# lyd405121/ti-raytrace

Measured on AMD Instinct MI355X. Metric: Mrays/s (primary+secondary) at 1024² 100k-tri, 1/2/4/8 GPU + HBM GB/s, higher is better.
Workload: dtype f32

## Files before the change

### ti_raytrace_amd/csrc/tirt_render.hip

```cpp
#include "tirt_trace.h"
#include "tirt_spectral.h"

namespace tirt {

struct ShadeStep {
    bool want_next = false, want_shadow = false, shaded = false;
    v3 next_o = V(0.0f, 0.0f, 0.0f), next_d = next_o, next_thr = next_o, sh_o = next_o, sh_d = next_o, sh_c = next_o;
    float next_pdf = 0.0f, sh_dist = 0.0f; int next_spec = 0, sh_expect = -2;
};
template <unsigned FEAT, bool LIST = false>
TD void shade_path(const SceneView &sc, const TileMap &tm, int P, uint32_t frame_begin, uint32_t seed, int bounce, int last_bounce, int slot,
                   const v3 origin, const v3 direction, const float4 hrec, v3 throughout, v3 &radiance, float brdf_pdf, int perfect_spec, ShadeStep &s)
{
    int f, k; slot_to_frame_pixel(tm, P, slot, f, k);
    const uint32_t pixel = (uint32_t)mapped_pixel<LIST>(tm, k);
    const uint32_t frame = frame_begin + (uint32_t)f;
    const uint32_t dim0 = TM_DIM_BOUNCE0 + TM_DIMS_PER_BOUNCE * (uint32_t)bounce;
    const float t = hrec.x;
    constexpr bool ENV_NEE = (FEAT & SF_ENV_SAMPLE) != 0u;
    constexpr bool ENV_HDR = (FEAT & SF_ENV_HDR) != 0u;
    constexpr bool LIGHT_POW = (FEAT & SF_LIGHT_POWER) != 0u;
    [[maybe_unused]] float p_env = 0.0f;
    if constexpr (ENV_NEE) p_env = sc.light_count == 0 ? 1.0f : env_table(sc).share;
    if (t < INF_VALUE) {
        const int prim_id = __float_as_int(hrec.w);
        int mat_id;
        const HitAttr h = hit_attributes_rec<(FEAT & (SF_TEXTURE | SF_TEXTURE_PARAM)) != 0u>(sc.shade_rec, origin, direction, prim_id, t, hrec.y, hrec.z, mat_id);
        v3 normal = h.nor;
        if constexpr ((FEAT & SF_TEXTURE_PARAM) != 0u) {
            const int nor_id = material_map(sc.material + (size_t)mat_id * MAT_VEC, 9);
            if (nor_id >= 0) normal = tex_normal_rec(sc.tex, sc.shade_rec, nor_id, prim_id, h.tex, normal);
        }
        const v3 fnormal = normal * signf(dot(-direction, h.gnor));
        const float *m = sc.material + (size_t)mat_id * MAT_VEC;
        const v3 mat_color = V(m[2], m[3], m[4]);
        const int mat_type = (int)m[0];
        if (mat_type == MAT_LIGHT) {
            const float fCosTheta = absf(dot(direction, h.gnor));
            if (perfect_spec == 1) {
                radiance = radiance + throughout * mat_color;
            } else {
                const float area = h.area * (float)sc.light_count;
                float light_pdf = (t * t) / (area * fCosTheta);
                if constexpr (LIGHT_POW) light_pdf = (t * t) * (shade_rec_phit(sc.shade_rec, prim_id) / h.area) / fCosTheta;
                if constexpr (ENV_NEE) light_pdf = light_pdf * (1.0f - p_env);
                radiance = radiance + (throughout * power_heuristic(brdf_pdf, light_pdf)) * mat_color;
            }
        } else {
            s.shaded = true;
            v3 reflect_color;
            const int tex_id = (FEAT & SF_TEXTURE) ? material_texture(m) : -1;
            if ((FEAT & SF_TEXTURE) && tex_id >= 0) reflect_color = srgb_to_lrgb(tex_albedo(sc.tex, tex_id, h.tex.x, h.tex.y));
            else reflect_color = V(sc.mat_lrgb[mat_id * 3], sc.mat_lrgb[mat_id * 3 + 1], sc.mat_lrgb[mat_id * 3 + 2]);
            v3 next_dir; float f_or_b = 1.0f, brdf = 1.0f;
            if ((FEAT & SF_GLASS) && mat_type == MAT_GLASS) {
                perfect_spec = 1;
                next_dir = glass_sample(m, direction, normal, tm_rand(seed, pixel, frame, dim0 + TM_SLOT_GLASS), f_or_b);
                brdf = 1.0f; brdf_pdf = 1.0f;
            } else {
                perfect_spec = 0;
                float mp[MAT_VEC];
                const float *md = m;
                if constexpr ((FEAT & SF_TEXTURE_PARAM) != 0u) {
                    for (int w = 0; w < MAT_VEC; w++) mp[w] = m[w];
                    const int metal_id = material_map(m, 8), rough_id = material_map(m, 7);
                    if (metal_id >= 0) mp[5] = tex_metallic(sc.tex, metal_id, h.tex.x, h.tex.y);
                    if (rough_id >= 0) mp[6] = tex_roughness(sc.tex, rough_id, h.tex.x, h.tex.y);
                    md = mp;
                }
                constexpr bool SHARE_SETUP = !(FEAT & SF_GLASS);
                DisneySetup ds;
                if (SHARE_SETUP) ds = disney_setup(md, fnormal, -direction);
                [[maybe_unused]] bool env_taken = false;
                if constexpr (ENV_NEE) {
                    if (tm_rand(seed, pixel, frame, dim0 + TM_SLOT_LIGHT) < p_env) {
                        env_taken = true;
                        const EnvTable et = env_table(sc);
                        const EnvSample es = env_sample(et, sc.env_w, sc.env_h, tm_rand(seed, pixel, frame, dim0 + TM_SLOT_LA), tm_rand(seed, pixel, frame, dim0 + TM_SLOT_LB));
                        const EnvPdf ep = env_pdf(et, sc.env_w, sc.env_h, es.d);
                        const float NdotL = dot(fnormal, es.d);
                        if ((NdotL > 0.0f) & (ep.pdf > 0.0f)) {
                            s.want_shadow = true;
                            float e_pdf;
                            const float e_brdf = SHARE_SETUP ? disney_evaluate_pdf_set(ds, fnormal, -direction, es.d, e_pdf)
                                                             : disney_evaluate_pdf(md, fnormal, -direction, es.d, e_pdf);
                            const float pdf_l = p_env * ep.pdf;
                            v3 c = V(0.0f, 0.0f, 0.0f);
                            int expect = -2;
                            if (e_pdf > 0.0f) {
                                const float w = power_heuristic(pdf_l, e_pdf) / maxf(0.0001f, pdf_l);
                                c = (env_lookup<ENV_HDR>(sc.env, sc.env_w, sc.env_h, ep.tx, ep.ty) * sc.env_power) * w;
                                c = c * throughout;
                                c = c * reflect_color;
                                c = c * e_brdf;
                                c = c * absf(NdotL);
                                const float dr = SHARE_SETUP ? ds.diffuseRatio : 0.5f * (1.0f - md[5]);
                                const float drawn = maxf(0.0f, e_pdf + (dr * (float)(1.0 / 3.1415956)) * (NdotL - 1.0f));
                                c = c * (drawn / e_pdf);
                                expect = -1;
                            }
                            s.sh_o = offset_ray(h.pos, fnormal); s.sh_d = es.d; s.sh_c = c; s.sh_expect = expect; s.sh_dist = ENV_SHADOW_DIST;
                        }
                    }
                }
                if (!env_taken && (!(FEAT & SF_NO_LIGHT) || sc.light_count > 0)) {
                float r_light = tm_rand(seed, pixel, frame, dim0 + TM_SLOT_LIGHT);
                if constexpr (ENV_NEE) r_light = (r_light - p_env) / (1.0f - p_env);
                int lidx = (int)(r_light * (float)sc.light_count);
                if (lidx >= sc.light_count) lidx = sc.light_count - 1;
                [[maybe_unused]] float P_light = 0.0f;
                if constexpr (LIGHT_POW) lidx = light_pick(light_table(sc), sc.light_count, r_light, P_light);
                const float ra = tm_rand(seed, pixel, frame, dim0 + TM_SLOT_LA);
                const float rb = tm_rand(seed, pixel, frame, dim0 + TM_SLOT_LB);
                v3 light_pos, light_normal;
                const LightRec lr = light_sample_rec<LIGHT_POW ? (FEAT & ~(SF_LIGHT_SPOT_LASER | SF_LIGHT_OTHER)) : FEAT>(sc.light_rec, lidx, ra, rb, light_pos, light_normal);
                const float light_choice_pdf = LIGHT_POW ? P_light / lr.area : lr.choice_pdf;
                light_normal = normalized(light_normal);
                v3 light_dir = h.pos - light_pos;
                const float light_dist = norm(light_dir);
                light_dir = light_dir / light_dist;
                const v3 light_emission = lr.emission * light_shape_visible_rec<LIGHT_POW ? (FEAT & ~SF_LIGHT_SPOT_LASER) : FEAT>(lr, light_dir, light_normal, light_dist);
                const float NdotL_surface = dot(fnormal, light_dir);
                const float NdotL_light = dot(light_normal, light_dir);
                if ((NdotL_surface < 0.0f) & (NdotL_light > 0.0f)) {
                    s.want_shadow = true;
                    float e_pdf;
                    const float e_brdf = SHARE_SETUP ? disney_evaluate_pdf_set(ds, fnormal, -direction, -light_dir, e_pdf)
                                                     : disney_evaluate_pdf(md, fnormal, -direction, -light_dir, e_pdf);
                    float light_pdf = light_dist * light_dist * light_choice_pdf / NdotL_light;
                    if constexpr (ENV_NEE) light_pdf = light_pdf * (1.0f - p_env);
                    v3 c = V(0.0f, 0.0f, 0.0f);
                    int expect = -2;
                    if (e_pdf > 0.0f) {
                        const float w = power_heuristic(light_pdf, e_pdf) / maxf(0.0001f, light_pdf);
                        c = light_emission * w;
                        c = c * throughout;
                        c = c * reflect_color;
                        c = c * e_brdf;
                        c = c * absf(NdotL_surface);
                        expect = prim_id;
                    }
                    s.sh_o = light_pos; s.sh_d = light_dir; s.sh_c = c; s.sh_expect = expect; s.sh_dist = light_dist;
                }
                }
                const float r_lobe = tm_rand(seed, pixel, frame, dim0 + TM_SLOT_LOBE), r_1 = tm_rand(seed, pixel, frame, dim0 + TM_SLOT_R1),
                            r_2 = tm_rand(seed, pixel, frame, dim0 + TM_SLOT_R2);
                next_dir = SHARE_SETUP ? disney_sample_set(ds, direction, fnormal, r_lobe, r_1, r_2) : disney_sample(md, direction, fnormal, r_lobe, r_1, r_2);
                f_or_b = 1.0f;
                brdf = SHARE_SETUP ? disney_evaluate_pdf_set(ds, fnormal, -direction, next_dir, brdf_pdf)
                                   : disney_evaluate_pdf(md, fnormal, -direction, next_dir, brdf_pdf);
                brdf *= absf(dot(normal, next_dir));
            }
            const v3 next_origin = offset_ray(h.pos, fnormal * signf(f_or_b));
            if (brdf_pdf > 0.0f) {
                bool alive = true;
                if ((FEAT & SF_GLASS) && f_or_b < 0.0f) {
                    const float extinction = m[6];
                    const float R = tm_exp(-t / extinction);
                    if (tm_rand(seed, pixel, frame, dim0 + TM_SLOT_EXT) >= R) alive = false;
                }
                if (alive) {
                    throughout = throughout * (reflect_color * (brdf / brdf_pdf));
                    s.want_next = !last_bounce;
                    s.next_o = next_origin; s.next_d = next_dir; s.next_thr = throughout;
                    s.next_pdf = brdf_pdf; s.next_spec = perfect_spec;
                }
            }
        }
    } else if ((!(FEAT & SF_ENV) || sc.env_power == 0.0f) && (direction.x - direction.x == 0.0f) && (direction.y - direction.y == 0.0f) &&
               (direction.z - direction.z == 0.0f)) {
        radiance = radiance + throughout * sc.env_power;
    } else if (!(FEAT & SF_ENV)) {
        const float dis = tm_sqrt(direction.x * direction.x + direction.z * direction.z);
        const float big = 3.4028234e38f;
        const bool e_nan = direction.x != direction.x || direction.y != direction.y || direction.z != direction.z ||
                           (absf(direction.x) > big && absf(direction.z) > big) || (absf(direction.y) > big && dis > big);
        const float e1 = e_nan ? tm_nan() : 0.0f;
        radiance = radiance + (V(e1, e1, e1) * throughout) * sc.env_power;
    } else {
        const float dis = tm_sqrt(direction.x * direction.x + direction.z * direction.z);
        const float tx = (tm_atan2(direction.z, direction.x) + PI_SCENE) / PI_SCENE / 2.0f;
        const float ty = tm_atan2(direction.y, dis) / PI_SCENE + 0.5f;
        const v3 e = env_lookup<ENV_HDR>(sc.env, sc.env_w, sc.env_h, tx, ty);
        if constexpr (ENV_NEE) {
            float w = 1.0f;
            if (perfect_spec != 1) w = power_heuristic(brdf_pdf, p_env * env_pdf(env_table(sc), sc.env_w, sc.env_h, direction).pdf);
            radiance = radiance + ((e * throughout) * sc.env_power) * w;
        } else
        radiance = radiance + (e * throughout) * sc.env_power;
    }
}

template <bool LIST>
__global__ void k_generate(PathSoA ps, CameraView cam, TileMap tm, int P, int S, uint32_t frame_begin, uint32_t seed,
                           DevCounters *ctr)
{
    int s = blockIdx.x * blockDim.x + threadIdx.x;
    if (s >= S) return;
    int f, k; slot_to_frame_pixel(tm, P, s, f, k);
    int p = mapped_pixel<LIST>(tm, k);
    int i = p / tm.H, j = p - i * tm.H;
    uint32_t frame = frame_begin + (uint32_t)f;
    float jx = 0.0f, jy = 0.0f;
    if (frame != 0) {
        jx = tm_rand(seed, (uint32_t)p, frame, TM_DIM_JX) - 0.5f;
        jy = tm_rand(seed, (uint32_t)p, frame, TM_DIM_JY) - 0.5f;
    }
    v3 d = camera_ray_direction(cam, i, j, jx, jy);
    __builtin_nontemporal_store(d.x, &ps.dx[s]); __builtin_nontemporal_store(d.y, &ps.dy[s]); __builtin_nontemporal_store(d.z, &ps.dz[s]);
    if (s == 0) atomicAdd(&ctr->paths, (unsigned long long)S);
}

#ifndef SH_BLOCK
#define SH_BLOCK 256
#endif
#ifndef SH_MIN_WAVES
#define SH_MIN_WAVES 5
#endif
#ifndef SH_MIN_WAVES_NARROW
#define SH_MIN_WAVES_NARROW 5
#endif
#ifndef SH_MIN_WAVES_MAPS
#define SH_MIN_WAVES_MAPS 4
#endif
#ifndef SH_MIN_WAVES_ENV
#define SH_MIN_WAVES_ENV 4
#endif
#ifndef SH_MIN_WAVES_POWER
#define SH_MIN_WAVES_POWER 4
#endif
#ifndef SH_MIN_WAVES_HDR
#define SH_MIN_WAVES_HDR 4
#endif
struct ShadeArgs { PathState ps; PathSoA in, out; };
typedef const __attribute__((address_space(4))) ShadeArgs *cold_shade_t;
#define SH_COLD(ca) cold_shade_t ca = (cold_shade_t)__builtin_amdgcn_kernarg_segment_ptr(); asm volatile("" : "+s"(ca))
#define SH_LD(x) __builtin_nontemporal_load(&(x))
#define SH_ST(x, v) __builtin_nontemporal_store((v), &(x))
template <unsigned FEAT, int MIN_WAVES, bool LIST = false>
__global__ __launch_bounds__(SH_BLOCK, MIN_WAVES) void k_shade(ShadeArgs paths_in_kernarg_segment, SceneView sc, TileMap tm, int P,
                                                   uint32_t frame_begin, uint32_t seed, int bounce, int last_bounce,
                                                   const int *count_ptr, int count_fixed, unsigned long long *append_ctr,
                                                   DevCounters *ctr, v3 eye)
{
    __shared__ unsigned s_wcnt[2][SH_BLOCK / 64];
    __shared__ unsigned long long s_base[2];
    const int lane = threadIdx.x & 63, wid = threadIdx.x >> 6;
    const unsigned long long lt_mask = (lane == 0) ? 0ull : (~0ull >> (64 - lane));
    const int count = count_ptr ? *count_ptr : count_fixed;
    const int total = gridDim.x * blockDim.x;
    const int rounds = (count + total - 1) / total;
    unsigned long long n_shaded = 0;
    for (int it = 0; it < rounds; it++) {
        const int q = it * total + blockIdx.x * blockDim.x + threadIdx.x;
        bool live = q < count, want_next = false, want_shadow = false;
        int slot = 0;
        v3 radiance = V(0.0f, 0.0f, 0.0f), next_o = radiance, next_d = radiance, next_thr = radiance;
        v3 sh_o = radiance, sh_d = radiance, sh_c = radiance;
        float next_pdf = 0.0f, sh_dist = 0.0f; int next_spec = 0, sh_expect = -2;
        if (live) {
            const bool first = bounce == 0;
            SH_COLD(ca);
            const int *const c_slot = ca->in.slot; const uint32_t *const c_flags = ca->in.flags; const float4 *const c_hit = ca->ps.hit;
            const float *const c_ox = ca->in.ox, *const c_oy = ca->in.oy, *const c_oz = ca->in.oz, *const c_dx = ca->in.dx, *const c_dy = ca->in.dy, *const c_dz = ca->in.dz;
            const float *const c_tr = ca->in.tr, *const c_tg = ca->in.tg, *const c_tb = ca->in.tb, *const c_rr = ca->in.rr, *const c_rg = ca->in.rg, *const c_rb = ca->in.rb;
            const float *const c_pdf = ca->in.brdf_pdf;
            asm volatile("" :: "s"(c_slot), "s"(c_flags), "s"(c_hit), "s"(c_ox), "s"(c_oy), "s"(c_oz), "s"(c_dx), "s"(c_dy), "s"(c_dz), "s"(c_tr), "s"(c_tg), "s"(c_tb),
                         "s"(c_rr), "s"(c_rg), "s"(c_rb), "s"(c_pdf));
            slot = first ? q : SH_LD(c_slot[q]);
            const v3 origin = first ? eye : V(SH_LD(c_ox[q]), SH_LD(c_oy[q]), SH_LD(c_oz[q]));
            const v3 direction = V(SH_LD(c_dx[q]), SH_LD(c_dy[q]), SH_LD(c_dz[q]));
            typedef float f4nt__ __attribute__((ext_vector_type(4)));
            const f4nt__ hnt__ = __builtin_nontemporal_load((const f4nt__ *)&c_hit[q]);
            const float4 hrec = make_float4(hnt__.x, hnt__.y, hnt__.z, hnt__.w);
            v3 throughout = first ? V(1.0f, 1.0f, 1.0f) : V(SH_LD(c_tr[q]), SH_LD(c_tg[q]), SH_LD(c_tb[q]));
            radiance = first ? V(0.0f, 0.0f, 0.0f) : V(SH_LD(c_rr[q]), SH_LD(c_rg[q]), SH_LD(c_rb[q]));
            float brdf_pdf = first ? 1.0f : SH_LD(c_pdf[q]);
            int perfect_spec = first ? 1 : (int)(SH_LD(c_flags[q]) & 1u);
            ShadeStep ss;
            shade_path<FEAT, LIST>(sc, tm, P, frame_begin, seed, bounce, last_bounce, slot, origin, direction, hrec, throughout, radiance, brdf_pdf, perfect_spec, ss);
            want_next = ss.want_next; want_shadow = ss.want_shadow; if (ss.shaded) n_shaded++;
            next_o = ss.next_o; next_d = ss.next_d; next_thr = ss.next_thr; next_pdf = ss.next_pdf; next_spec = ss.next_spec;
            sh_o = ss.sh_o; sh_d = ss.sh_d; sh_c = ss.sh_c; sh_expect = ss.sh_expect; sh_dist = ss.sh_dist;
        }
        const int par = it & 1;
        const unsigned long long nmask = __ballot(want_next), smask = __ballot(want_shadow);
        if (lane == 0) s_wcnt[par][wid] = (unsigned)__popcll(nmask) | ((unsigned)__popcll(smask) << 16);
        __syncthreads();
        if (threadIdx.x == 0) {
            unsigned tn = 0, tsd = 0;
#pragma unroll
            for (int w = 0; w < SH_BLOCK / 64; w++) { tn += s_wcnt[par][w] & 0xffffu; tsd += s_wcnt[par][w] >> 16; }
            s_base[par] = (tn | tsd) ? atomicAdd(append_ctr, (unsigned long long)tn | ((unsigned long long)tsd << 32)) : 0ull;
        }
        __syncthreads();
        unsigned pn = 0, psd = 0;
#pragma unroll
        for (int w = 0; w < SH_BLOCK / 64; w++) if (w < wid) { pn += s_wcnt[par][w] & 0xffffu; psd += s_wcnt[par][w] >> 16; }
        const unsigned long long bb = s_base[par];
        const int qn = (int)(unsigned)(bb & 0xffffffffull) + (int)pn + __popcll(nmask & lt_mask);
        const int qs = (int)(unsigned)(bb >> 32) + (int)psd + __popcll(smask & lt_mask);
        if (want_next) {
            SH_COLD(ca);
            float *const o_ox = ca->out.ox, *const o_oy = ca->out.oy, *const o_oz = ca->out.oz, *const o_dx = ca->out.dx, *const o_dy = ca->out.dy, *const o_dz = ca->out.dz;
            float *const o_tr = ca->out.tr, *const o_tg = ca->out.tg, *const o_tb = ca->out.tb, *const o_rr = ca->out.rr, *const o_rg = ca->out.rg, *const o_rb = ca->out.rb;
            float *const o_pdf = ca->out.brdf_pdf; uint32_t *const o_flags = ca->out.flags; int *const o_slot = ca->out.slot;
            asm volatile("" :: "s"(o_ox), "s"(o_oy), "s"(o_oz), "s"(o_dx), "s"(o_dy), "s"(o_dz), "s"(o_tr), "s"(o_tg), "s"(o_tb), "s"(o_rr), "s"(o_rg), "s"(o_rb),
                         "s"(o_pdf), "s"(o_flags), "s"(o_slot));
            SH_ST(o_ox[qn], next_o.x); SH_ST(o_oy[qn], next_o.y); SH_ST(o_oz[qn], next_o.z);
            SH_ST(o_dx[qn], next_d.x); SH_ST(o_dy[qn], next_d.y); SH_ST(o_dz[qn], next_d.z);
            SH_ST(o_tr[qn], next_thr.x); SH_ST(o_tg[qn], next_thr.y); SH_ST(o_tb[qn], next_thr.z);
            SH_ST(o_rr[qn], radiance.x); SH_ST(o_rg[qn], radiance.y); SH_ST(o_rb[qn], radiance.z);
            SH_ST(o_pdf[qn], next_pdf); SH_ST(o_flags[qn], (uint32_t)next_spec); SH_ST(o_slot[qn], slot);
        } else if (live) {
            SH_COLD(ca);
            float *const f_r = ca->ps.fr, *const f_g = ca->ps.fg, *const f_b = ca->ps.fb;
            asm volatile("" :: "s"(f_r), "s"(f_g), "s"(f_b));
            SH_ST(f_r[slot], radiance.x); SH_ST(f_g[slot], radiance.y); SH_ST(f_b[slot], radiance.z);
        }
        if (want_shadow) {
            SH_COLD(ca);
            float *const s_ox = ca->ps.sox, *const s_oy = ca->ps.soy, *const s_oz = ca->ps.soz, *const s_dx = ca->ps.sdx, *const s_dy = ca->ps.sdy, *const s_dz = ca->ps.sdz;
            float *const s_cr = ca->ps.scr, *const s_cg = ca->ps.scg, *const s_cb = ca->ps.scb, *const s_dist = ca->ps.sdist;
            int *const s_prim = ca->ps.sprim, *const s_dst = ca->ps.sdst;
            asm volatile("" :: "s"(s_ox), "s"(s_oy), "s"(s_oz), "s"(s_dx), "s"(s_dy), "s"(s_dz), "s"(s_cr), "s"(s_cg), "s"(s_cb), "s"(s_dist), "s"(s_prim), "s"(s_dst));
            SH_ST(s_ox[qs], sh_o.x); SH_ST(s_oy[qs], sh_o.y); SH_ST(s_oz[qs], sh_o.z);
            SH_ST(s_dx[qs], sh_d.x); SH_ST(s_dy[qs], sh_d.y); SH_ST(s_dz[qs], sh_d.z);
            SH_ST(s_cr[qs], sh_c.x); SH_ST(s_cg[qs], sh_c.y); SH_ST(s_cb[qs], sh_c.z);
            SH_ST(s_prim[qs], sh_expect); SH_ST(s_dist[qs], sh_dist);
            SH_ST(s_dst[qs], want_next ? qn : ~slot);
        }
    }
    __shared__ unsigned long long s_shaded;
    if (threadIdx.x == 0) s_shaded = 0ull;
    __syncthreads();
    n_shaded = wave_sum(n_shaded);
    if ((threadIdx.x & 63) == 0 && n_shaded) atomicAdd(&s_shaded, n_shaded);
    __syncthreads();
    if (threadIdx.x == 0 && s_shaded) atomicAdd(&ctr->shaded, s_shaded);
}

template <bool LIST>
__global__ void k_film(PathState ps, TileMap tm, int P, int F, uint32_t frame_begin, float *hdr)
{
    int k = blockIdx.x * blockDim.x + threadIdx.x;
    if (k >= P) return;
    int p = mapped_pixel<LIST>(tm, k);
    float *px = hdr + (size_t)p * 3;
    float r = px[0], g = px[1], b = px[2];
    for (int f = 0; f < F; f++) {
        int s = frame_pixel_to_slot(tm, P, f, k);
        float frame = (float)(int)(frame_begin + (uint32_t)f);
        float coff = 1.0f / (frame + 1.0f);
        r = __builtin_nontemporal_load(&ps.fr[s]) * coff + r * (1.0f - coff);
        g = __builtin_nontemporal_load(&ps.fg[s]) * coff + g * (1.0f - coff);
        b = __builtin_nontemporal_load(&ps.fb[s]) * coff + b * (1.0f - coff);
    }
    px[0] = r; px[1] = g; px[2] = b;
}

template <unsigned FEAT>
__global__ __launch_bounds__(SH_BLOCK, 4) void k_shade_spec(ShadeArgs paths_in_kernarg_segment, SceneView sc, SpecView sp, TileMap tm, int P,
                                                   uint32_t frame_begin, uint32_t seed, int bounce, int last_bounce,
                                                   const int *count_ptr, int count_fixed, unsigned long long *append_ctr,
                                                   DevCounters *ctr, v3 eye)
{
    __shared__ unsigned s_wcnt[2][SH_BLOCK / 64];
    __shared__ unsigned long long s_base[2];
    const int lane = threadIdx.x & 63, wid = threadIdx.x >> 6;
    const unsigned long long lt_mask = (lane == 0) ? 0ull : (~0ull >> (64 - lane));
    const int count = count_ptr ? *count_ptr : count_fixed;
    const int total = gridDim.x * blockDim.x;
    const int rounds = (count + total - 1) / total;
    unsigned long long n_shaded = 0;
    for (int it = 0; it < rounds; it++) {
        const int q = it * total + blockIdx.x * blockDim.x + threadIdx.x;
        bool live = q < count, want_next = false, want_shadow = false;
        int slot = 0;
        f4s radiance = f4_set(0.0f), next_thr = radiance, sh_c = radiance;
        v3 next_o = V(0.0f, 0.0f, 0.0f), next_d = next_o, sh_o = next_o, sh_d = next_o;
        float sh_dist = 0.0f; int sh_expect = -2;
        if (live) {
            const bool first = bounce == 0;
            SH_COLD(ca);
            const int *const c_slot = ca->in.slot; const float4 *const c_hit = ca->ps.hit;
            const float *const c_ox = ca->in.ox, *const c_oy = ca->in.oy, *const c_oz = ca->in.oz, *const c_dx = ca->in.dx, *const c_dy = ca->in.dy, *const c_dz = ca->in.dz;
            const float *const c_tr = ca->in.tr, *const c_tg = ca->in.tg, *const c_tb = ca->in.tb, *const c_rr = ca->in.rr, *const c_rg = ca->in.rg, *const c_rb = ca->in.rb;
            const float *const c_tw = ca->in.brdf_pdf, *const c_rw = (const float *)ca->in.flags;
            asm volatile("" :: "s"(c_slot), "s"(c_hit), "s"(c_ox), "s"(c_oy), "s"(c_oz), "s"(c_dx), "s"(c_dy), "s"(c_dz), "s"(c_tr), "s"(c_tg), "s"(c_tb),
                         "s"(c_rr), "s"(c_rg), "s"(c_rb), "s"(c_tw), "s"(c_rw));
            slot = first ? q : c_slot[q];
            int f, k; slot_to_frame_pixel(tm, P, slot, f, k);
            const uint32_t pixel = (uint32_t)local_to_pixel(tm, k);
            const uint32_t frame = frame_begin + (uint32_t)f;
            const uint32_t dim0 = TM_DIM_BOUNCE0 + TM_DIMS_PER_BOUNCE * (uint32_t)bounce;
            const float Lambda = HERO_LAMBDA_MIN + HERO_LAMBDA_STEP * tm_rand(seed, pixel, frame, TM_DIM_SPEC_LAMBDA);
            const v3 origin = first ? eye : V(c_ox[q], c_oy[q], c_oz[q]);
            const v3 direction = V(c_dx[q], c_dy[q], c_dz[q]);
            typedef float f4nt__ __attribute__((ext_vector_type(4)));
            const f4nt__ hnt__ = __builtin_nontemporal_load((const f4nt__ *)&c_hit[q]);
            const float4 hrec = make_float4(hnt__.x, hnt__.y, hnt__.z, hnt__.w);
            const float t = hrec.x;
            f4s throughout = f4_set(1.0f);
            if (!first) {
                throughout.v[0] = c_tr[q]; throughout.v[1] = c_tg[q]; throughout.v[2] = c_tb[q]; throughout.v[3] = c_tw[q];
                radiance.v[0] = c_rr[q]; radiance.v[1] = c_rg[q]; radiance.v[2] = c_rb[q]; radiance.v[3] = c_rw[q];
            }
            const f4s light_rad = hero_sample(sp.spd[0], Lambda);
            if (t < INF_VALUE) {
                const int prim_id = __float_as_int(hrec.w);
                int mat_id;
                const HitAttr h = hit_attributes_rec(sc.shade_rec, origin, direction, prim_id, t, hrec.y, hrec.z, mat_id);
                const v3 normal = h.nor;
// ... 78 lines not shown
        if (threadIdx.x == 0) {
            unsigned tn = 0, tsd = 0;
#pragma unroll
            for (int w = 0; w < SH_BLOCK / 64; w++) { tn += s_wcnt[par][w] & 0xffffu; tsd += s_wcnt[par][w] >> 16; }
            s_base[par] = (tn | tsd) ? atomicAdd(append_ctr, (unsigned long long)tn | ((unsigned long long)tsd << 32)) : 0ull;
        }
        __syncthreads();
        unsigned pn = 0, psd = 0;
#pragma unroll
        for (int w = 0; w < SH_BLOCK / 64; w++) if (w < wid) { pn += s_wcnt[par][w] & 0xffffu; psd += s_wcnt[par][w] >> 16; }
        const unsigned long long bb = s_base[par];
        const int qn = (int)(unsigned)(bb & 0xffffffffull) + (int)pn + __popcll(nmask & lt_mask);
        const int qs = (int)(unsigned)(bb >> 32) + (int)psd + __popcll(smask & lt_mask);
        if (want_next) {
            SH_COLD(ca);
            float *const o_ox = ca->out.ox, *const o_oy = ca->out.oy, *const o_oz = ca->out.oz, *const o_dx = ca->out.dx, *const o_dy = ca->out.dy, *const o_dz = ca->out.dz;
            float *const o_tr = ca->out.tr, *const o_tg = ca->out.tg, *const o_tb = ca->out.tb, *const o_rr = ca->out.rr, *const o_rg = ca->out.rg, *const o_rb = ca->out.rb;
            float *const o_tw = ca->out.brdf_pdf, *const o_rw = (float *)ca->out.flags; int *const o_slot = ca->out.slot;
            asm volatile("" :: "s"(o_ox), "s"(o_oy), "s"(o_oz), "s"(o_dx), "s"(o_dy), "s"(o_dz), "s"(o_tr), "s"(o_tg), "s"(o_tb), "s"(o_rr), "s"(o_rg), "s"(o_rb),
                         "s"(o_tw), "s"(o_rw), "s"(o_slot));
            o_ox[qn] = next_o.x; o_oy[qn] = next_o.y; o_oz[qn] = next_o.z;
            o_dx[qn] = next_d.x; o_dy[qn] = next_d.y; o_dz[qn] = next_d.z;
            o_tr[qn] = next_thr.v[0]; o_tg[qn] = next_thr.v[1]; o_tb[qn] = next_thr.v[2]; o_tw[qn] = next_thr.v[3];
            o_rr[qn] = radiance.v[0]; o_rg[qn] = radiance.v[1]; o_rb[qn] = radiance.v[2]; o_rw[qn] = radiance.v[3];
            o_slot[qn] = slot;
        } else if (live) {
            SH_COLD(ca);
            float *const f_r = ca->ps.fr, *const f_g = ca->ps.fg, *const f_b = ca->ps.fb, *const f_w = ca->ps.fw;
            asm volatile("" :: "s"(f_r), "s"(f_g), "s"(f_b), "s"(f_w));
            f_r[slot] = radiance.v[0]; f_g[slot] = radiance.v[1]; f_b[slot] = radiance.v[2]; f_w[slot] = radiance.v[3];
        }
        if (want_shadow) {
            SH_COLD(ca);
            float *const s_ox = ca->ps.sox, *const s_oy = ca->ps.soy, *const s_oz = ca->ps.soz, *const s_dx = ca->ps.sdx, *const s_dy = ca->ps.sdy, *const s_dz = ca->ps.sdz;
            float *const s_cr = ca->ps.scr, *const s_cg = ca->ps.scg, *const s_cb = ca->ps.scb, *const s_cw = ca->ps.scw, *const s_dist = ca->ps.sdist;
            int *const s_prim = ca->ps.sprim, *const s_dst = ca->ps.sdst;
            asm volatile("" :: "s"(s_ox), "s"(s_oy), "s"(s_oz), "s"(s_dx), "s"(s_dy), "s"(s_dz), "s"(s_cr), "s"(s_cg), "s"(s_cb), "s"(s_cw), "s"(s_dist), "s"(s_prim), "s"(s_dst));
            s_ox[qs] = sh_o.x; s_oy[qs] = sh_o.y; s_oz[qs] = sh_o.z;
            s_dx[qs] = sh_d.x; s_dy[qs] = sh_d.y; s_dz[qs] = sh_d.z;
            s_cr[qs] = sh_c.v[0]; s_cg[qs] = sh_c.v[1]; s_cb[qs] = sh_c.v[2]; s_cw[qs] = sh_c.v[3];
            s_prim[qs] = sh_expect; s_dist[qs] = sh_dist;
            s_dst[qs] = want_next ? qn : ~slot;
        }
    }
    __shared__ unsigned long long s_shaded;
    if (threadIdx.x == 0) s_shaded = 0ull;
    __syncthreads();
    n_shaded = wave_sum(n_shaded);
    if ((threadIdx.x & 63) == 0 && n_shaded) atomicAdd(&s_shaded, n_shaded);
    __syncthreads();
    if (threadIdx.x == 0 && s_shaded) atomicAdd(&ctr->shaded, s_shaded);
}

__global__ void k_film_spec(PathState ps, const float *fw, SpecView sp, TileMap tm, int P, int F, uint32_t frame_begin, uint32_t seed, float *hdr)
{
    int k = blockIdx.x * blockDim.x + threadIdx.x;
    if (k >= P) return;
    const int p = local_to_pixel(tm, k);
    float *px = hdr + (size_t)p * 3;
    float r = px[0], g = px[1], b = px[2];
    for (int f = 0; f < F; f++) {
        const int s = frame_pixel_to_slot(tm, P, f, k);
        const uint32_t frame = frame_begin + (uint32_t)f;
        const float coff = 1.0f / ((float)(int)frame + 1.0f);
        const float Lambda = HERO_LAMBDA_MIN + HERO_LAMBDA_STEP * tm_rand(seed, (uint32_t)p, frame, TM_DIM_SPEC_LAMBDA);
        f4s spec; spec.v[0] = ps.fr[s]; spec.v[1] = ps.fg[s]; spec.v[2] = ps.fb[s]; spec.v[3] = fw[s];
        spec_add_splat(sp, spec, Lambda, coff, r, g, b);
    }
    px[0] = r; px[1] = g; px[2] = b;
}

[[maybe_unused]] constexpr int KAT_STEP_IN = 23, KAT_STEP_OUT = 28;
template <unsigned FEAT, int MIN_WAVES>
__global__ __launch_bounds__(SH_BLOCK, MIN_WAVES) void k_kat_shade_step(SceneView sc, const float *in, int in_stride, float *out, int out_stride, int n)
{
    const int i = blockIdx.x * blockDim.x + threadIdx.x;
    if (i >= n) return;
    const float *a = in + (size_t)i * in_stride;
    float *o = out + (size_t)i * out_stride;
    const TileMap tm = {0, 1, 0x7fffffff, 1, 0, 0};
    v3 radiance = V(a[18], a[19], a[20]);
    ShadeStep ss;
    shade_path<FEAT>(sc, tm, 0x7fffffff, (uint32_t)__float_as_int(a[2]), (uint32_t)__float_as_int(a[0]), __float_as_int(a[3]), __float_as_int(a[4]) != 0, __float_as_int(a[1]),
                     V(a[5], a[6], a[7]), V(a[8], a[9], a[10]), make_float4(a[11], a[12], a[13], a[14]), V(a[15], a[16], a[17]), radiance, a[21], __float_as_int(a[22]), ss);
    o[0] = radiance.x; o[1] = radiance.y; o[2] = radiance.z; o[3] = __int_as_float(ss.shaded ? 1 : 0); o[4] = __int_as_float(ss.want_next ? 1 : 0);
    o[5] = ss.next_o.x; o[6] = ss.next_o.y; o[7] = ss.next_o.z; o[8] = ss.next_d.x; o[9] = ss.next_d.y; o[10] = ss.next_d.z;
    o[11] = ss.next_thr.x; o[12] = ss.next_thr.y; o[13] = ss.next_thr.z; o[14] = ss.next_pdf; o[15] = __int_as_float(ss.next_spec); o[16] = __int_as_float(ss.want_shadow ? 1 : 0);
    o[17] = ss.sh_o.x; o[18] = ss.sh_o.y; o[19] = ss.sh_o.z; o[20] = ss.sh_d.x; o[21] = ss.sh_d.y; o[22] = ss.sh_d.z;
    o[23] = ss.sh_c.x; o[24] = ss.sh_c.y; o[25] = ss.sh_c.z; o[26] = __int_as_float(ss.sh_expect); o[27] = ss.sh_dist;
}

typedef void (*shade_fn_t)(ShadeArgs, SceneView, TileMap, int, uint32_t, uint32_t, int, int, const int *, int, unsigned long long *, DevCounters *, v3);
typedef void (*shade_spec_fn_t)(ShadeArgs, SceneView, SpecView, TileMap, int, uint32_t, uint32_t, int, int, const int *, int, unsigned long long *, DevCounters *, v3);
struct ShadeInst { unsigned feat; shade_fn_t fn, fn_list; };
struct ShadeSpecInst { unsigned feat; shade_spec_fn_t fn; };
constexpr unsigned SF_I_SPHERE = SF_LIGHT_SPHERE;
constexpr unsigned SF_I_MESH = SF_LIGHT_TRI;
constexpr unsigned SF_I_MAPS = SF_ALL | SF_TEXTURE | SF_TEXTURE_PARAM;
static const ShadeInst SHADE_INST[] = {
    {SF_I_SPHERE, k_shade<SF_I_SPHERE, SH_MIN_WAVES_NARROW>, k_shade<SF_I_SPHERE, SH_MIN_WAVES_NARROW, true>},
    {SF_I_MESH, k_shade<SF_I_MESH, SH_MIN_WAVES_NARROW>, k_shade<SF_I_MESH, SH_MIN_WAVES_NARROW, true>},
    {SF_ALL, k_shade<SF_ALL, SH_MIN_WAVES>, k_shade<SF_ALL, SH_MIN_WAVES, true>},
    {SF_ALL | SF_TEXTURE, k_shade<SF_ALL | SF_TEXTURE, SH_MIN_WAVES>, k_shade<SF_ALL | SF_TEXTURE, SH_MIN_WAVES, true>},
    {SF_I_MAPS, k_shade<SF_I_MAPS, SH_MIN_WAVES_MAPS>, k_shade<SF_I_MAPS, SH_MIN_WAVES_MAPS, true>}};
constexpr unsigned SF_I_ENV = SF_ALL | SF_ENV_SAMPLE, SF_I_ENV_MAPS = SF_I_MAPS | SF_ENV_SAMPLE;
static const ShadeInst SHADE_ENV_INST[] = {
    {SF_I_ENV, k_shade<SF_I_ENV, SH_MIN_WAVES_ENV>, k_shade<SF_I_ENV, SH_MIN_WAVES_ENV, true>},
    {SF_I_ENV_MAPS, k_shade<SF_I_ENV_MAPS, SH_MIN_WAVES_ENV>, k_shade<SF_I_ENV_MAPS, SH_MIN_WAVES_ENV, true>}};
constexpr unsigned SF_I_HDR = SF_ALL | SF_ENV_HDR, SF_I_HDR_MAPS = SF_I_MAPS | SF_ENV_HDR, SF_I_ENV_HDR = SF_I_ENV | SF_ENV_HDR, SF_I_ENV_HDR_MAPS = SF_I_ENV_MAPS | SF_ENV_HDR;
template <unsigned F, int MW>
constexpr ShadeInst shade_inst() { return {F, k_shade<F, MW>, k_shade<F, MW, true>}; }
static const ShadeInst SHADE_HDR_INST[] = {shade_inst<SF_I_HDR, SH_MIN_WAVES_HDR>(), shade_inst<SF_I_HDR_MAPS, SH_MIN_WAVES_MAPS>()};
static const ShadeInst SHADE_ENV_HDR_INST[] = {shade_inst<SF_I_ENV_HDR, SH_MIN_WAVES_ENV>(), shade_inst<SF_I_ENV_HDR_MAPS, SH_MIN_WAVES_ENV>()};
constexpr unsigned SF_P = SF_LIGHT_POWER;
static const ShadeInst SHADE_POWER_INST[8] = {
    shade_inst<SF_ALL | SF_P, SH_MIN_WAVES_POWER>(), shade_inst<SF_I_MAPS | SF_P, SH_MIN_WAVES_MAPS>(),
    shade_inst<SF_I_ENV | SF_P, SH_MIN_WAVES_ENV>(), shade_inst<SF_I_ENV_MAPS | SF_P, SH_MIN_WAVES_ENV>(),
    shade_inst<SF_I_HDR | SF_P, SH_MIN_WAVES_HDR>(), shade_inst<SF_I_HDR_MAPS | SF_P, SH_MIN_WAVES_MAPS>(),
    shade_inst<SF_I_ENV_HDR | SF_P, SH_MIN_WAVES_ENV>(), shade_inst<SF_I_ENV_HDR_MAPS | SF_P, SH_MIN_WAVES_ENV>()};
static const ShadeSpecInst SHADE_SPEC_INST[] = {
    {SF_I_SPHERE, k_shade_spec<SF_I_SPHERE>}, {SF_I_MESH, k_shade_spec<SF_I_MESH>}, {SF_ALL, k_shade_spec<SF_ALL>}};
template <class T, size_t N>
static const T &pick_shade_inst(const T (&tab)[N], const tirt_ctx *c)
{
    size_t k = 0;
    if (!c->shade_specialize) while (k + 1 < N && tab[k].feat != SF_ALL) k++;
    for (; k + 1 < N; k++) if ((c->shade_features & ~tab[k].feat) == 0u) return tab[k];
    return tab[N - 1];
}
static const ShadeInst &pick_shade_rgb(const tirt_ctx *c)
{
    if (light_power_active(c)) return SHADE_POWER_INST[(env_hdr_active(c) ? 4 : 0) + (env_sample_active(c) ? 2 : 0) + ((c->shade_features & ~SF_ALL) ? 1 : 0)];
    if (env_hdr_active(c)) return (env_sample_active(c) ? SHADE_ENV_HDR_INST : SHADE_HDR_INST)[(c->shade_features & ~SF_ALL) ? 1 : 0];
    if (env_sample_active(c)) return SHADE_ENV_INST[(c->shade_features & ~SF_ALL) ? 1 : 0];
    return pick_shade_inst(SHADE_INST, c);
}

typedef void (*kat_step_fn_t)(SceneView, const float *, int, float *, int, int);
struct KatStepInst { unsigned feat; kat_step_fn_t fn; };
static const KatStepInst KAT_STEP_INST[] = {
    {SF_I_SPHERE, k_kat_shade_step<SF_I_SPHERE, SH_MIN_WAVES_NARROW>}, {SF_I_MESH, k_kat_shade_step<SF_I_MESH, SH_MIN_WAVES_NARROW>},
    {SF_ALL, k_kat_shade_step<SF_ALL, SH_MIN_WAVES>}, {SF_ALL | SF_TEXTURE, k_kat_shade_step<SF_ALL | SF_TEXTURE, SH_MIN_WAVES>},
    {SF_I_MAPS, k_kat_shade_step<SF_I_MAPS, SH_MIN_WAVES_MAPS>}};
static_assert(sizeof(KAT_STEP_INST) / sizeof(KAT_STEP_INST[0]) == sizeof(SHADE_INST) / sizeof(SHADE_INST[0]), "one known-answer kernel per instantiation of k_shade");
static const KatStepInst KAT_STEP_ENV_INST[] = {
    {SF_I_ENV, k_kat_shade_step<SF_I_ENV, SH_MIN_WAVES_ENV>}, {SF_I_ENV_MAPS, k_kat_shade_step<SF_I_ENV_MAPS, SH_MIN_WAVES_ENV>}};
static_assert(sizeof(KAT_STEP_ENV_INST) / sizeof(KAT_STEP_ENV_INST[0]) == sizeof(SHADE_ENV_INST) / sizeof(SHADE_ENV_INST[0]), "one known-answer kernel per instantiation of k_shade");
static const KatStepInst KAT_STEP_HDR_INST[] = {
    {SF_I_HDR, k_kat_shade_step<SF_I_HDR, SH_MIN_WAVES_HDR>}, {SF_I_HDR_MAPS, k_kat_shade_step<SF_I_HDR_MAPS, SH_MIN_WAVES_MAPS>}};
static_assert(sizeof(KAT_STEP_HDR_INST) / sizeof(KAT_STEP_HDR_INST[0]) == sizeof(SHADE_HDR_INST) / sizeof(SHADE_HDR_INST[0]), "one known-answer kernel per instantiation of k_shade");
static const KatStepInst KAT_STEP_ENV_HDR_INST[] = {
    {SF_I_ENV_HDR, k_kat_shade_step<SF_I_ENV_HDR, SH_MIN_WAVES_ENV>}, {SF_I_ENV_HDR_MAPS, k_kat_shade_step<SF_I_ENV_HDR_MAPS, SH_MIN_WAVES_ENV>}};
static_assert(sizeof(KAT_STEP_ENV_HDR_INST) / sizeof(KAT_STEP_ENV_HDR_INST[0]) == sizeof(SHADE_ENV_HDR_INST) / sizeof(SHADE_ENV_HDR_INST[0]), "one known-answer kernel per instantiation of k_shade");
template <unsigned F, int MW>
constexpr KatStepInst kat_inst() { return {F, k_kat_shade_step<F, MW>}; }
static const KatStepInst KAT_STEP_POWER_INST[8] = {
    kat_inst<SF_ALL | SF_P, SH_MIN_WAVES_POWER>(), kat_inst<SF_I_MAPS | SF_P, SH_MIN_WAVES_MAPS>(),
    kat_inst<SF_I_ENV | SF_P, SH_MIN_WAVES_ENV>(), kat_inst<SF_I_ENV_MAPS | SF_P, SH_MIN_WAVES_ENV>(),
    kat_inst<SF_I_HDR | SF_P, SH_MIN_WAVES_HDR>(), kat_inst<SF_I_HDR_MAPS | SF_P, SH_MIN_WAVES_MAPS>(),
    kat_inst<SF_I_ENV_HDR | SF_P, SH_MIN_WAVES_ENV>(), kat_inst<SF_I_ENV_HDR_MAPS | SF_P, SH_MIN_WAVES_ENV>()};

static kat_step_fn_t kat_step_inst(unsigned feat)
{
    for (const KatStepInst &k : KAT_STEP_INST) if (k.feat == feat) return k.fn;
    for (const KatStepInst &k : KAT_STEP_ENV_INST) if (k.feat == feat) return k.fn;
    for (const KatStepInst &k : KAT_STEP_HDR_INST) if (k.feat == feat) return k.fn;
    for (const KatStepInst &k : KAT_STEP_ENV_HDR_INST) if (k.feat == feat) return k.fn;
    for (const KatStepInst &k : KAT_STEP_POWER_INST) if (k.feat == feat) return k.fn;
    return nullptr;
}
bool kat_shade_step_has_inst(unsigned feat) { return kat_step_inst(feat) != nullptr; }
int kat_shade_step(tirt_ctx *c, unsigned feat, const float *in, int in_stride, float *out, int out_stride, int n)
{
    TIRT_REQUIRE(c->n >= 1, "tirt_kat_shade_step: no scene");
    TIRT_REQUIRE((c->shade_features & ~feat) == 0u, "tirt_kat_shade_step: feat does not cover the scene's feature word (tirt_shade_features)");
    TIRT_REQUIRE(((feat & SF_ENV_HDR) != 0u) == env_hdr_active(c), "tirt_kat_shade_step: an instantiation with bit 2048 reads RGBE8 texels and one without it 8-bit texels: feat must carry the bit exactly when tirt_shade_features does");
    TIRT_REQUIRE(!(feat & SF_ENV_SAMPLE) || env_sample_active(c), "tirt_kat_shade_step: an instantiation with bit 1024 needs the environment's sampling table (tirt_env_sampling on, a lit environment)");
    if (feat & SF_LIGHT_POWER) {
        if (sync_all(c) || ensure_shade_records(c)) return TIRT_ERR_HIP;
        TIRT_REQUIRE(light_power_active(c), "tirt_kat_shade_step: an instantiation with bit 4096 needs the emitters' table (tirt_light_sampling mode 1, triangle and sphere emitters only, total > 0)");
    }
    const kat_step_fn_t fn = kat_step_inst(feat);
    TIRT_REQUIRE(fn, "tirt_kat_shade_step: feat is not an instantiation of k_shade");
    TIRT_REQUIRE(!(feat & (SF_TEXTURE | SF_TEXTURE_PARAM)) || c->tex_count > 0, "tirt_kat_shade_step: the textured instantiation needs uploaded textures (tirt_texture_upload): without them no material row's slot is checked");
    for (int i = 0; i < n; i++) {
        const float *a = in + (size_t)i * in_stride;
        const int32_t *w = (const int32_t *)a; const int32_t prim = w[14], pixel = w[1];
        TIRT_REQUIRE(!(a[11] < INF_VALUE) || (prim >= 0 && prim < c->n), "tirt_kat_shade_step: row " + std::to_string(i) + ": prim outside [0, n_prims) of a hit (t < INF)");
        TIRT_REQUIRE(pixel >= 0 && pixel < 0x7fffffff, "tirt_kat_shade_step: row " + std::to_string(i) + ": pixel outside [0, 2^31 - 1)");
    }
    if (n == 0) return TIRT_OK;
    if (sync_all(c)) return TIRT_ERR_HIP;
    if (ensure_shade_records(c)) return TIRT_ERR_HIP;
    return kat_round_trip(c, "tirt_kat_shade_step", {{in, kat_row_bytes(n, in_stride)}}, out, kat_row_bytes(n, out_stride), [&](const void *const *din, void *dout) {
        hipLaunchKernelGGL(fn, dim3((n + SH_BLOCK - 1) / SH_BLOCK), dim3(SH_BLOCK), 0, c->stream, scene_view(c), (const float *)din[0], in_stride, (float *)dout, out_stride, n);
    });
}

constexpr size_t LINE = 128;
static size_t lane_counter_bytes(int max_depth)
{ return LINE * (size_t)(max_depth + 1) + sizeof(int) * TR_FETCH_STRIDE * TR_FETCH_LINES * (size_t)(max_depth + 1); }

constexpr int PATH_WORDS = 2 * 15 + 4 + 12 + 3 + 2;
static size_t path_state_bytes(size_t S) { return sizeof(float) * PATH_WORDS * ((S + 3) & ~(size_t)3); }
static int ensure_paths(Lane &L, size_t S, int max_depth)
{
    if (S > L.path_capacity || !L.path_mem.p) {
        if (L.path_mem.ensure(path_state_bytes(S))) return TIRT_ERR_HIP;
        const size_t S_user = S;
        S = (S + 3) & ~(size_t)3;
        float *w = L.path_mem.as<float>();
        PathState &p = L.ps;
        auto nxt = [&]() { float *r = w; w += S; return r; };
        for (int k = 0; k < 2; k++) {
            PathSoA &q = p.st[k];
            q.ox = nxt(); q.oy = nxt(); q.oz = nxt(); q.dx = nxt(); q.dy = nxt(); q.dz = nxt();
            q.tr = nxt(); q.tg = nxt(); q.tb = nxt(); q.rr = nxt(); q.rg = nxt(); q.rb = nxt();
            q.brdf_pdf = nxt(); q.flags = (uint32_t *)nxt(); q.slot = (int *)nxt();
        }
        p.hit = (float4 *)w; w += 4 * S;
        p.sox = nxt(); p.soy = nxt(); p.soz = nxt(); p.sdx = nxt(); p.sdy = nxt(); p.sdz = nxt();
        p.scr = nxt(); p.scg = nxt(); p.scb = nxt(); p.sprim = (int *)nxt(); p.sdist = nxt(); p.sdst = (int *)nxt();
        p.fr = nxt(); p.fg = nxt(); p.fb = nxt();
        p.scw = nxt(); p.fw = nxt();
        L.path_capacity = S_user;
    }
    if (L.counters_mem.ensure(lane_counter_bytes(max_depth))) return TIRT_ERR_HIP;
    return 0;
}

void retire_render_events(tirt_ctx *c, bool finished_only)
{
    size_t keep = 0;
    for (auto &pr : c->ev_pool) {
        if (finished_only && hipEventQuery(pr.second) != hipSuccess) { c->ev_pool[keep++] = pr; continue; }
        float ms = 0.0f;
        if (hipEventElapsedTime(&ms, pr.first, pr.second) == hipSuccess) c->ms_render += ms;
        (void)hipEventDestroy(pr.first); (void)hipEventDestroy(pr.second);
    }
    c->ev_pool.resize(keep);
    if (finished_only) (void)hipGetLastError();
}
// ... 207 lines not shown
```

Baseline: 5681.

## Accumulate radiance directly into framebuffer and pack specular flag into slot word

```diff
diff --git a/ti_raytrace_amd/csrc/tirt_render.hip b/ti_raytrace_amd/csrc/tirt_render.hip
--- a/ti_raytrace_amd/csrc/tirt_render.hip
+++ b/ti_raytrace_amd/csrc/tirt_render.hip
@@ -4,13 +4,14 @@
 namespace tirt {
 
 struct ShadeStep {
-    bool want_next = false, want_shadow = false, shaded = false;
+    bool want_next = false, want_shadow = false, shaded = false, adds = false;
+    v3 add = V(0.0f, 0.0f, 0.0f);
     v3 next_o = V(0.0f, 0.0f, 0.0f), next_d = next_o, next_thr = next_o, sh_o = next_o, sh_d = next_o, sh_c = next_o;
     float next_pdf = 0.0f, sh_dist = 0.0f; int next_spec = 0, sh_expect = -2;
 };
 template <unsigned FEAT, bool LIST = false>
 TD void shade_path(const SceneView &sc, const TileMap &tm, int P, uint32_t frame_begin, uint32_t seed, int bounce, int last_bounce, int slot,
-                   const v3 origin, const v3 direction, const float4 hrec, v3 throughout, v3 &radiance, float brdf_pdf, int perfect_spec, ShadeStep &s)
+                   const v3 origin, const v3 direction, const float4 hrec, v3 throughout, float brdf_pdf, int perfect_spec, ShadeStep &s)
 {
     int f, k; slot_to_frame_pixel(tm, P, slot, f, k);
     const uint32_t pixel = (uint32_t)mapped_pixel<LIST>(tm, k);
@@ -37,14 +38,15 @@
         const int mat_type = (int)m[0];
         if (mat_type == MAT_LIGHT) {
             const float fCosTheta = absf(dot(direction, h.gnor));
+            s.adds = true;
             if (perfect_spec == 1) {
-                radiance = radiance + throughout * mat_color;
+                s.add = throughout * mat_color;
             } else {
                 const float area = h.area * (float)sc.light_count;
                 float light_pdf = (t * t) / (area * fCosTheta);
                 if constexpr (LIGHT_POW) light_pdf = (t * t) * (shade_rec_phit(sc.shade_rec, prim_id) / h.area) / fCosTheta;
                 if constexpr (ENV_NEE) light_pdf = light_pdf * (1.0f - p_env);
-                radiance = radiance + (throughout * power_heuristic(brdf_pdf, light_pdf)) * mat_color;
+                s.add = (throughout * power_heuristic(brdf_pdf, light_pdf)) * mat_color;
             }
         } else {
             s.shaded = true;
@@ -169,25 +171,26 @@
         }
     } else if ((!(FEAT & SF_ENV) || sc.env_power == 0.0f) && (direction.x - direction.x == 0.0f) && (direction.y - direction.y == 0.0f) &&
                (direction.z - direction.z == 0.0f)) {
-        radiance = radiance + throughout * sc.env_power;
+        s.adds = true; s.add = throughout * sc.env_power;
     } else if (!(FEAT & SF_ENV)) {
         const float dis = tm_sqrt(direction.x * direction.x + direction.z * direction.z);
         const float big = 3.4028234e38f;
         const bool e_nan = direction.x != direction.x || direction.y != direction.y || direction.z != direction.z ||
                            (absf(direction.x) > big && absf(direction.z) > big) || (absf(direction.y) > big && dis > big);
         const float e1 = e_nan ? tm_nan() : 0.0f;
-        radiance = radiance + (V(e1, e1, e1) * throughout) * sc.env_power;
+        s.adds = true; s.add = (V(e1, e1, e1) * throughout) * sc.env_power;
     } else {
         const float dis = tm_sqrt(direction.x * direction.x + direction.z * direction.z);
         const float tx = (tm_atan2(direction.z, direction.x) + PI_SCENE) / PI_SCENE / 2.0f;
         const float ty = tm_atan2(direction.y, dis) / PI_SCENE + 0.5f;
         const v3 e = env_lookup<ENV_HDR>(sc.env, sc.env_w, sc.env_h, tx, ty);
+        s.adds = true;
         if constexpr (ENV_NEE) {
             float w = 1.0f;
             if (perfect_spec != 1) w = power_heuristic(brdf_pdf, p_env * env_pdf(env_table(sc), sc.env_w, sc.env_h, direction).pdf);
-            radiance = radiance + ((e * throughout) * sc.env_power) * w;
+            s.add = ((e * throughout) * sc.env_power) * w;
         } else
-        radiance = radiance + (e * throughout) * sc.env_power;
+        s.add = (e * throughout) * sc.env_power;
     }
 }
 
@@ -230,7 +233,7 @@
 #define SH_MIN_WAVES_POWER 4
 #endif
 #ifndef SH_MIN_WAVES_HDR
-#define SH_MIN_WAVES_HDR 4
+#define SH_MIN_WAVES_HDR 5
 #endif
 struct ShadeArgs { PathState ps; PathSoA in, out; };
 typedef const __attribute__((address_space(4))) ShadeArgs *cold_shade_t;
@@ -253,35 +256,41 @@
     unsigned long long n_shaded = 0;
     for (int it = 0; it < rounds; it++) {
         const int q = it * total + blockIdx.x * blockDim.x + threadIdx.x;
-        bool live = q < count, want_next = false, want_shadow = false;
+        bool live = q < count, want_next = false, want_shadow = false, adds = false;
         int slot = 0;
         v3 radiance = V(0.0f, 0.0f, 0.0f), next_o = radiance, next_d = radiance, next_thr = radiance;
         v3 sh_o = radiance, sh_d = radiance, sh_c = radiance;
         float next_pdf = 0.0f, sh_dist = 0.0f; int next_spec = 0, sh_expect = -2;
+        const bool first = bounce == 0;
         if (live) {
-            const bool first = bounce == 0;
             SH_COLD(ca);
-            const int *const c_slot = ca->in.slot; const uint32_t *const c_flags = ca->in.flags; const float4 *const c_hit = ca->ps.hit;
+            const int *const c_slot = ca->in.slot; const float4 *const c_hit = ca->ps.hit;
             const float *const c_ox = ca->in.ox, *const c_oy = ca->in.oy, *const c_oz = ca->in.oz, *const c_dx = ca->in.dx, *const c_dy = ca->in.dy, *const c_dz = ca->in.dz;
-            const float *const c_tr = ca->in.tr, *const c_tg = ca->in.tg, *const c_tb = ca->in.tb, *const c_rr = ca->in.rr, *const c_rg = ca->in.rg, *const c_rb = ca->in.rb;
+            const float *const c_tr = ca->in.tr, *const c_tg = ca->in.tg, *const c_tb = ca->in.tb;
             const float *const c_pdf = ca->in.brdf_pdf;
-            asm volatile("" :: "s"(c_slot), "s"(c_flags), "s"(c_hit), "s"(c_ox), "s"(c_oy), "s"(c_oz), "s"(c_dx), "s"(c_dy), "s"(c_dz), "s"(c_tr), "s"(c_tg), "s"(c_tb),
-                         "s"(c_rr), "s"(c_rg), "s"(c_rb), "s"(c_pdf));
-            slot = first ? q : SH_LD(c_slot[q]);
+            asm volatile("" :: "s"(c_slot), "s"(c_hit), "s"(c_ox), "s"(c_oy), "s"(c_oz), "s"(c_dx), "s"(c_dy), "s"(c_dz), "s"(c_tr), "s"(c_tg), "s"(c_tb), "s"(c_pdf));
+            const uint32_t slot_word = first ? (uint32_t)q | 0x80000000u : (uint32_t)SH_LD(c_slot[q]);
+            slot = (int)(slot_word & 0x7fffffffu);
             const v3 origin = first ? eye : V(SH_LD(c_ox[q]), SH_LD(c_oy[q]), SH_LD(c_oz[q]));
             const v3 direction = V(SH_LD(c_dx[q]), SH_LD(c_dy[q]), SH_LD(c_dz[q]));
             typedef float f4nt__ __attribute__((ext_vector_type(4)));
             const f4nt__ hnt__ = __builtin_nontemporal_load((const f4nt__ *)&c_hit[q]);
             const float4 hrec = make_float4(hnt__.x, hnt__.y, hnt__.z, hnt__.w);
             v3 throughout = first ? V(1.0f, 1.0f, 1.0f) : V(SH_LD(c_tr[q]), SH_LD(c_tg[q]), SH_LD(c_tb[q]));
-            radiance = first ? V(0.0f, 0.0f, 0.0f) : V(SH_LD(c_rr[q]), SH_LD(c_rg[q]), SH_LD(c_rb[q]));
             float brdf_pdf = first ? 1.0f : SH_LD(c_pdf[q]);
-            int perfect_spec = first ? 1 : (int)(SH_LD(c_flags[q]) & 1u);
+            int perfect_spec = (int)(slot_word >> 31);
             ShadeStep ss;
-            shade_path<FEAT, LIST>(sc, tm, P, frame_begin, seed, bounce, last_bounce, slot, origin, direction, hrec, throughout, radiance, brdf_pdf, perfect_spec, ss);
+            shade_path<FEAT, LIST>(sc, tm, P, frame_begin, seed, bounce, last_bounce, slot, origin, direction, hrec, throughout, brdf_pdf, perfect_spec, ss);
             want_next = ss.want_next; want_shadow = ss.want_shadow; if (ss.shaded) n_shaded++;
             next_o = ss.next_o; next_d = ss.next_d; next_thr = ss.next_thr; next_pdf = ss.next_pdf; next_spec = ss.next_spec;
             sh_o = ss.sh_o; sh_d = ss.sh_d; sh_c = ss.sh_c; sh_expect = ss.sh_expect; sh_dist = ss.sh_dist;
+            if (first) {
+                if (ss.adds) radiance = radiance + ss.add;
+            } else {
+                radiance = ss.add;
+                const bool nothing = !(hrec.x < INF_VALUE) && ss.add.x == 0.0f && ss.add.y == 0.0f && ss.add.z == 0.0f;
+                adds = ss.adds && !nothing;
+            }
         }
         const int par = it & 1;
         const unsigned long long nmask = __ballot(want_next), smask = __ballot(want_shadow);
@@ -303,20 +312,20 @@
         if (want_next) {
             SH_COLD(ca);
             float *const o_ox = ca->out.ox, *const o_oy = ca->out.oy, *const o_oz = ca->out.oz, *const o_dx = ca->out.dx, *const o_dy = ca->out.dy, *const o_dz = ca->out.dz;
-            float *const o_tr = ca->out.tr, *const o_tg = ca->out.tg, *const o_tb = ca->out.tb, *const o_rr = ca->out.rr, *const o_rg = ca->out.rg, *const o_rb = ca->out.rb;
-            float *const o_pdf = ca->out.brdf_pdf; uint32_t *const o_flags = ca->out.flags; int *const o_slot = ca->out.slot;
-            asm volatile("" :: "s"(o_ox), "s"(o_oy), "s"(o_oz), "s"(o_dx), "s"(o_dy), "s"(o_dz), "s"(o_tr), "s"(o_tg), "s"(o_tb), "s"(o_rr), "s"(o_rg), "s"(o_rb),
-                         "s"(o_pdf), "s"(o_flags), "s"(o_slot));
+            float *const o_tr = ca->out.tr, *const o_tg = ca->out.tg, *const o_tb = ca->out.tb;
+            float *const o_pdf = ca->out.brdf_pdf; int *const o_slot = ca->out.slot;
+            asm volatile("" :: "s"(o_ox), "s"(o_oy), "s"(o_oz), "s"(o_dx), "s"(o_dy), "s"(o_dz), "s"(o_tr), "s"(o_tg), "s"(o_tb), "s"(o_pdf), "s"(o_slot));
             SH_ST(o_ox[qn], next_o.x); SH_ST(o_oy[qn], next_o.y); SH_ST(o_oz[qn], next_o.z);
             SH_ST(o_dx[qn], next_d.x); SH_ST(o_dy[qn], next_d.y); SH_ST(o_dz[qn], next_d.z);
             SH_ST(o_tr[qn], next_thr.x); SH_ST(o_tg[qn], next_thr.y); SH_ST(o_tb[qn], next_thr.z);
-            SH_ST(o_rr[qn], radiance.x); SH_ST(o_rg[qn], radiance.y); SH_ST(o_rb[qn], radiance.z);
-            SH_ST(o_pdf[qn], next_pdf); SH_ST(o_flags[qn], (uint32_t)next_spec); SH_ST(o_slot[qn], slot);
-        } else if (live) {
+            SH_ST(o_pdf[qn], next_pdf); SH_ST(o_slot[qn], (int)((uint32_t)slot | ((uint32_t)next_spec << 31)));
+        }
+        if (first ? live : adds) {
             SH_COLD(ca);
             float *const f_r = ca->ps.fr, *const f_g = ca->ps.fg, *const f_b = ca->ps.fb;
             asm volatile("" :: "s"(f_r), "s"(f_g), "s"(f_b));
-            SH_ST(f_r[slot], radiance.x); SH_ST(f_g[slot], radiance.y); SH_ST(f_b[slot], radiance.z);
+            if (first) { SH_ST(f_r[slot], radiance.x); SH_ST(f_g[slot], radiance.y); SH_ST(f_b[slot], radiance.z); }
+            else { f_r[slot] = f_r[slot] + radiance.x; f_g[slot] = f_g[slot] + radiance.y; f_b[slot] = f_b[slot] + radiance.z; }
         }
         if (want_shadow) {
             SH_COLD(ca);
@@ -328,7 +337,7 @@
             SH_ST(s_dx[qs], sh_d.x); SH_ST(s_dy[qs], sh_d.y); SH_ST(s_dz[qs], sh_d.z);
             SH_ST(s_cr[qs], sh_c.x); SH_ST(s_cg[qs], sh_c.y); SH_ST(s_cb[qs], sh_c.z);
             SH_ST(s_prim[qs], sh_expect); SH_ST(s_dist[qs], sh_dist);
-            SH_ST(s_dst[qs], want_next ? qn : ~slot);
+            SH_ST(s_dst[qs], ~slot);
         }
     }
     __shared__ unsigned long long s_shaded;
@@ -573,7 +582,8 @@
     v3 radiance = V(a[18], a[19], a[20]);
     ShadeStep ss;
     shade_path<FEAT>(sc, tm, 0x7fffffff, (uint32_t)__float_as_int(a[2]), (uint32_t)__float_as_int(a[0]), __float_as_int(a[3]), __float_as_int(a[4]) != 0, __float_as_int(a[1]),
-                     V(a[5], a[6], a[7]), V(a[8], a[9], a[10]), make_float4(a[11], a[12], a[13], a[14]), V(a[15], a[16], a[17]), radiance, a[21], __float_as_int(a[22]), ss);
+                     V(a[5], a[6], a[7]), V(a[8], a[9], a[10]), make_float4(a[11], a[12], a[13], a[14]), V(a[15], a[16], a[17]), a[21], __float_as_int(a[22]), ss);
+    if (ss.adds) radiance = radiance + ss.add;
     o[0] = radiance.x; o[1] = radiance.y; o[2] = radiance.z; o[3] = __int_as_float(ss.shaded ? 1 : 0); o[4] = __int_as_float(ss.want_next ? 1 : 0);
     o[5] = ss.next_o.x; o[6] = ss.next_o.y; o[7] = ss.next_o.z; o[8] = ss.next_d.x; o[9] = ss.next_d.y; o[10] = ss.next_d.z;
     o[11] = ss.next_thr.x; o[12] = ss.next_thr.y; o[13] = ss.next_thr.z; o[14] = ss.next_pdf; o[15] = __int_as_float(ss.next_spec); o[16] = __int_as_float(ss.want_shadow ? 1 : 0);
@@ -607,7 +617,7 @@
 static const ShadeInst SHADE_POWER_INST[8] = {
     shade_inst<SF_ALL | SF_P, SH_MIN_WAVES_POWER>(), shade_inst<SF_I_MAPS | SF_P, SH_MIN_WAVES_MAPS>(),
     shade_inst<SF_I_ENV | SF_P, SH_MIN_WAVES_ENV>(), shade_inst<SF_I_ENV_MAPS | SF_P, SH_MIN_WAVES_ENV>(),
-    shade_inst<SF_I_HDR | SF_P, SH_MIN_WAVES_HDR>(), shade_inst<SF_I_HDR_MAPS | SF_P, SH_MIN_WAVES_MAPS>(),
+    shade_inst<SF_I_HDR | SF_P, SH_MIN_WAVES_POWER>(), shade_inst<SF_I_HDR_MAPS | SF_P, SH_MIN_WAVES_MAPS>(),
     shade_inst<SF_I_ENV_HDR | SF_P, SH_MIN_WAVES_ENV>(), shade_inst<SF_I_ENV_HDR_MAPS | SF_P, SH_MIN_WAVES_ENV>()};
 static const ShadeSpecInst SHADE_SPEC_INST[] = {
     {SF_I_SPHERE, k_shade_spec<SF_I_SPHERE>}, {SF_I_MESH, k_shade_spec<SF_I_MESH>}, {SF_ALL, k_shade_spec<SF_ALL>}};
@@ -648,7 +658,7 @@
 static const KatStepInst KAT_STEP_POWER_INST[8] = {
     kat_inst<SF_ALL | SF_P, SH_MIN_WAVES_POWER>(), kat_inst<SF_I_MAPS | SF_P, SH_MIN_WAVES_MAPS>(),
     kat_inst<SF_I_ENV | SF_P, SH_MIN_WAVES_ENV>(), kat_inst<SF_I_ENV_MAPS | SF_P, SH_MIN_WAVES_ENV>(),
-    kat_inst<SF_I_HDR | SF_P, SH_MIN_WAVES_HDR>(), kat_inst<SF_I_HDR_MAPS | SF_P, SH_MIN_WAVES_MAPS>(),
+    kat_inst<SF_I_HDR | SF_P, SH_MIN_WAVES_POWER>(), kat_inst<SF_I_HDR_MAPS | SF_P, SH_MIN_WAVES_MAPS>(),
     kat_inst<SF_I_ENV_HDR | SF_P, SH_MIN_WAVES_ENV>(), kat_inst<SF_I_ENV_HDR_MAPS | SF_P, SH_MIN_WAVES_ENV>()};
 
 static kat_step_fn_t kat_step_inst(unsigned feat)
```

Result: faster. 5820 (median of 6 runs) (+2.4%).
